# luigifcruz/radio-core

Hardware: AMD Instinct MI355X
Metric: IQ Msamples/s through Tuner+WBFM at 1024 channels (higher is better)
Workload: dtype f32

## Files before the change

### radio-core_amd/csrc/fft_kernel.h

```cpp
#pragma once

#include <hip/hip_runtime.h>

#include <cstdio>
#include <cstdlib>
#include <type_traits>

#include "fft_engine.h"
#include "tile_ns.h"

namespace rcfm {
RCFM_NS_OPEN
namespace fftk {

constexpr int W = RCFM_TILE_W;
constexpr int kLogW = W == 16 ? 4 : W == 8 ? 3 : 2;
static_assert((1 << kLogW) == W, "tile width: 4, 8 or 16 lines");
constexpr int kThreads = 256 * W / 16;

__device__ __forceinline__ float2 cmul(float2 a, float2 b) {
    typedef float v2f __attribute__((ext_vector_type(2)));
    v2f A, B, D;
    A.x = a.x; A.y = a.y; B.x = b.x; B.y = b.y;
    asm("v_pk_mul_f32 %0, %1, %2 op_sel:[0,0] op_sel_hi:[0,1]" : "=v"(D) : "v"(A), "v"(B));
// ... 765 lines not shown
    constexpr int kZeroFrom = kZeroQ > 0 && kZeroQ < R0 ? kZeroQ * (L / R0) : L;
    __shared__ __attribute__((aligned(16))) float2 tile[L * kRowsPitch];
    __shared__ __attribute__((aligned(16))) float2 tw[L];
    const FftPass& p1 = d1.p;
    const FftPass& p2 = d2.p;
    const int tid = threadIdx.x;
    const int w = tid & (W - 1), rg = tid >> kLogW;

    LineId id;
    const BlockPos bp = block_pos();
    id.batch = bp.batch;
    id.o1 = 0;
    id.o2 = 0;
    const int i0 = (int)bp.tile * W;
    const int left = (int)p1.n_inner - i0;
    const int wvalid = left < W ? left : W;
    const int64_t in_base = (int64_t)id.batch * d1.in_batch + (int64_t)i0 * p1.in_i;
    const int64_t mid_base = (int64_t)id.batch * d1.out_batch + i0;
    const int64_t out_base = (int64_t)id.batch * d2.out_batch + i0;
    const unsigned in_i = (unsigned)p1.in_i, mid_k = (unsigned)p1.out_k, out_k = (unsigned)p2.out_k;

    auto kbase = [](int g) -> int {
        if constexpr (S == 2) {
            return g;
        } else if constexpr (S == 3) {
            constexpr int w1 = L / (R0 * RL);
            const int q1 = g / w1, q2 = g - q1 * w1;
            return q1 + R0 * q2;
        } else {
            constexpr int w1 = L / (R0 * RL), w2 = L / (R0 * R1 * RL);
            const int q1 = g / w1, r1 = g - q1 * w1;
            const int q2 = r1 / w2, q3 = r1 - q2 * w2;
            return q1 + R0 * (q2 + R1 * q3);
        }
    };

    float2 v[nld];
#pragma unroll
    for (int it = 0; it < nld; ++it) {
        int e = tid + T * it;
        if ((L * W) % T != 0) e = e < L * W ? e : 0;
        const int wl = e / L, l = e - wl * L;
        const int wc = wl < wvalid ? wl : 0;
        id.i = i0 + wc;
        v[it] = load.fetch(id, l, in_base, (unsigned)wc * in_i + (unsigned)l);
    }
    float aux[nitL * RL];
    {
        const int wc = w < wvalid ? w : 0;
        id.i = i0 + wc;
#pragma unroll
        for (int it = 0; it < nitL; ++it) {
            int g = rg + RG * it;
            if (rowsL % RG != 0) g = g < rowsL ? g : 0;
            const int kb = kbase(g);
#pragma unroll
            for (int q = 0; q < RL; ++q) {
                const int k = kb + (L / RL) * q;
                aux[it * RL + q] = mid.fetch_aux(id, k, mid_base, (unsigned)k * mid_k + (unsigned)wc);
            }
        }
    }
    for (int e = tid; e < L; e += T) tw[e] = d1.stage_tw[e];

#pragma unroll
    for (int it = 0; it < nld; ++it) {
        const int e = tid + T * it;
        const int wl = e / L, l = e - wl * L;
        id.i = i0 + wl;
        float2 x = load.post(id, l, v[it]);
        if ((L * W) % T == 0 || e < L * W) tile[lds_slot<true>(l, wl)] = x;
    }
    lds_barrier();
    stage_lds<L, R0, L, true, RG>(tile, tw, w, rg);
    lds_barrier();
    if constexpr (S >= 3) {
        stage_lds<L, R1, L / R0, true, RG>(tile, tw, w, rg);
        lds_barrier();
    }
    if constexpr (S >= 4) {
        stage_lds<L, R2, L / (R0 * R1), true, RG>(tile, tw, w, rg);
        lds_barrier();
    }

    id.i = i0 + w;
    float2 xr[nitL * RL];
#pragma unroll
    for (int it = 0; it < nitL; ++it) {
        const int g = rg + RG * it;
        if ((rowsL % RG == 0) || g < rowsL) {
#pragma unroll
            for (int q = 0; q < RL; ++q) xr[it * RL + q] = tile[lds_slot<true>(g * RL + q, w)];
            dft_p<RL>(&xr[it * RL]);
        }
    }
    lds_barrier();
#pragma unroll
    for (int it = 0; it < nitL; ++it) {
        const int g = rg + RG * it;
        if ((rowsL % RG == 0) || g < rowsL) {
            const int kb = kbase(g);
#pragma unroll
            for (int q = 0; q < RL; ++q) {
                const int k = kb + (L / RL) * q;
                if constexpr (mid_upper_rows_zero<MidOp>::value) {
                    if ((L / RL) * q > L / 2) {
                        if ((L / RL) * q < kZeroFrom) tile[lds_slot<true>(k, w)] = make_float2(0.f, 0.f);
                        continue;
                    }
                }
                float2 y = mid(id, k, xr[it * RL + dft_slot<RL>(q)], aux[it * RL + q]);
                tile[lds_slot<true>(k, w)] = y;
            }
        }
    }
    lds_barrier();

    stage_lds<L, R0, L, true, RG, true, false, kZeroQ>(tile, tw, w, rg);
    lds_barrier();
    if constexpr (S >= 3) {
        stage_lds<L, R1, L / R0, true, RG>(tile, tw, w, rg);
        lds_barrier();
    }
    if constexpr (S >= 4) {
        stage_lds<L, R2, L / (R0 * R1), true, RG>(tile, tw, w, rg);
        lds_barrier();
    }
    const bool lane_ok = w < wvalid;
    const unsigned f = (unsigned)((int64_t)(i0 + w) * p2.tw_i);
    const float2 D = big_twiddle(d2, f * (unsigned)(L / RL));
#pragma unroll
    for (int it = 0; it < nitL; ++it) {
        const int g = rg + RG * it;
        if ((rowsL % RG == 0) || g < rowsL) {
            float2 x[RL];
#pragma unroll
            for (int q = 0; q < RL; ++q) x[q] = tile[lds_slot<true>(g * RL + q, w)];
            dft_p<RL>(x);
            const int kb = kbase(g);
            float2 Tw = big_twiddle(d2, f * (unsigned)kb);
            if (lane_ok) {
#pragma unroll
                for (int q = 0; q < RL; ++q) {
                    const int k = kb + (L / RL) * q;
                    const float2 y = cmul(x[dft_slot<RL>(q)], Tw);
                    Tw = cmul(Tw, D);
                    store(id, k, out_base, (unsigned)k * out_k + (unsigned)w, y);
                }
            }
        }
    }
}

template <int L, int R0, int R1, int R2, int R3, int T, class LoadOp, class MidOp, class StoreOp>
__global__ __launch_bounds__(T, (T * 16 / W >= 512 ? 4 : 1)) void k_fft_tile2_pair(FftPassDev d1, FftPassDev d2, LoadOp load,
                                                                          MidOp mid, StoreOp store, int count) {
    constexpr int S = (R0 > 1) + (R1 > 1) + (R2 > 1) + (R3 > 1);
    static_assert(S >= 2 && R0 * R1 * R2 * R3 == L, "bad radix list");
    constexpr int RL = (S == 2) ? R1 : (S == 3) ? R2 : R3;
    constexpr int RG = T / W;
    constexpr int nld = (L * W + T - 1) / T;
    constexpr int rowsL = L / RL, nitL = (rowsL + RG - 1) / RG;
    __shared__ __attribute__((aligned(16))) float2 tile[L * kRowsPitch];
    __shared__ __attribute__((aligned(16))) float2 tw[L];
    const FftPass& p1 = d1.p;
    const FftPass& p2 = d2.p;
    const int tid = threadIdx.x;
    const int w = tid & (W - 1), rg = tid >> kLogW;

    LineId id;
    const BlockPos bp = block_pos();
    id.batch = bp.batch;
    id.o1 = 0;
    id.o2 = 0;
    const int c0 = 2 * (int)bp.batch;
    const bool has1 = c0 + 1 < count;
    const int c1 = has1 ? c0 + 1 : c0;
    const int i0 = (int)bp.tile * W;
    const int left = (int)p1.n_inner - i0;
    const int wvalid = left < W ? left : W;
    const int64_t in_base = (int64_t)id.batch * d1.in_batch + (int64_t)i0 * p1.in_i;
    const int blk16 = mid.blk16;
    const int64_t mid_tile = blk16 ? (int64_t)(i0 >> 4) * blk16 + (i0 & 15) : (int64_t)i0;
    const int64_t mid_base0 = (int64_t)c0 * (blk16 ? mid.stride : d1.out_batch) + mid_tile;
    const int64_t mid_base1 = (int64_t)c1 * (blk16 ? mid.stride : d1.out_batch) + mid_tile;
    const int64_t out_base0 = (int64_t)c0 * d2.out_batch + i0;
    const int64_t out_base1 = (int64_t)c1 * d2.out_batch + i0;
    const unsigned in_i = (unsigned)p1.in_i, mid_k = blk16 ? 16u : (unsigned)p1.out_k, out_k = (unsigned)p2.out_k;
    const int wc = w < wvalid ? w : 0;

    auto lane_off = [&](int it) -> unsigned {
        int g = rg + RG * it;
        if (rowsL % RG != 0) g = g < rowsL ? g : 0;
        return (unsigned)last_stage_base<L, R0, R1, RL, S>(g) * mid_k + (unsigned)wc;
    };
    auto q_off = [&](int q) -> int64_t { return (int64_t)((L / RL) * q) * mid_k; };

    float2 v[nld];
#pragma unroll
    for (int it = 0; it < nld; ++it) {
        int e = tid + T * it;
        if ((L * W) % T != 0) e = e < L * W ? e : 0;
        const int wl = e / L, l = e - wl * L;
        const int wcl = wl < wvalid ? wl : 0;
        id.i = i0 + wcl;
        v[it] = load.fetch(id, l, in_base, (unsigned)wcl * in_i + (unsigned)l);
    }
    for (int e = tid; e < L; e += T) tw[e] = d1.stage_tw[e];
#pragma unroll
    for (int it = 0; it < nld; ++it) {
        const int e = tid + T * it;
        const int wl = e / L, l = e - wl * L;
        id.i = i0 + wl;
        const float2 x = load.post(id, l, v[it]);
        if ((L * W) % T == 0 || e < L * W) tile[lds_slot<true>(l, wl)] = x;
    }
    lds_barrier();
    stage_lds<L, R0, L, true, RG>(tile, tw, w, rg);
    lds_barrier();
    if constexpr (S >= 3) {
        stage_lds<L, R1, L / R0, true, RG>(tile, tw, w, rg);
        lds_barrier();
    }
    if constexpr (S >= 4) {
        stage_lds<L, R2, L / (R0 * R1), true, RG>(tile, tw, w, rg);
        lds_barrier();
    }

    using In0 = decltype(mid.fetch0(mid_base0, mid_base1, 0u));
    In0 a0[nitL * RL];
#pragma unroll
    for (int it = 0; it < nitL; ++it)
#pragma unroll
        for (int q = 0; q < RL; ++q)
            a0[it * RL + q] = mid.fetch0(mid_base0 + q_off(q), mid_base1 + q_off(q), lane_off(it));

    id.i = i0 + w;
    using Keep = typename MidOp::Keep;
    float2 u0[nitL * RL];
    Keep keep[nitL * RL];
#pragma unroll
    for (int it = 0; it < nitL; ++it) {
        const int g = rg + RG * it;
        if ((rowsL % RG == 0) || g < rowsL) {
            float2 x[RL];
#pragma unroll
            for (int q = 0; q < RL; ++q) x[q] = tile[lds_slot<true>(g * RL + q, w)];
            dft_p<RL>(x);
#pragma unroll
            for (int q = 0; q < RL; ++q)
                u0[it * RL + q] = mid.first(x[dft_slot<RL>(q)], a0[it * RL + q], keep[it * RL + q]);
        }
        __builtin_amdgcn_sched_barrier(0);
    }
    lds_barrier();
#pragma unroll
    for (int it = 0; it < nitL; ++it) {
        const int g = rg + RG * it;
        if ((rowsL % RG == 0) || g < rowsL) {
            const int kb = last_stage_base<L, R0, R1, RL, S>(g);
#pragma unroll
            for (int q = 0; q < RL; ++q) tile[lds_slot<true>(kb + (L / RL) * q, w)] = u0[it * RL + q];
        }
    }
    lds_barrier();

    const unsigned f = (unsigned)((int64_t)(i0 + w) * p2.tw_i);
    const float2 D = big_twiddle(d2, f * (unsigned)(L / RL));
    const bool lane_ok = w < wvalid;
    auto second_transform = [&](int64_t out_base) {
        stage_lds<L, R0, L, true, RG>(tile, tw, w, rg);
        lds_barrier();
        if constexpr (S >= 3) {
            stage_lds<L, R1, L / R0, true, RG>(tile, tw, w, rg);
            lds_barrier();
        }
        if constexpr (S >= 4) {
            stage_lds<L, R2, L / (R0 * R1), true, RG>(tile, tw, w, rg);
            lds_barrier();
        }
#pragma unroll
        for (int it = 0; it < nitL; ++it) {
            const int g = rg + RG * it;
            if ((rowsL % RG == 0) || g < rowsL) {
                float2 x[RL];
#pragma unroll
                for (int q = 0; q < RL; ++q) x[q] = tile[lds_slot<true>(g * RL + q, w)];
                dft_p<RL>(x);
                const int kb = last_stage_base<L, R0, R1, RL, S>(g);
                float2 Tw = big_twiddle(d2, f * (unsigned)kb);
                if (lane_ok) {
#pragma unroll
                    for (int q = 0; q < RL; ++q) {
                        const int k = kb + (L / RL) * q;
                        const float2 y = cmul(x[dft_slot<RL>(q)], Tw);
                        Tw = cmul(Tw, D);
                        store(id, k, out_base, (unsigned)k * out_k + (unsigned)w, y);
                    }
                }
            }
        }
    };

    float a1[nitL * RL];
#pragma unroll
    for (int it = 0; it < nitL; ++it)
#pragma unroll
        for (int q = 0; q < RL; ++q) a1[it * RL + q] = mid.fetch1(mid_base1 + q_off(q), lane_off(it));

    second_transform(out_base0);
    if (!has1) return;
    lds_barrier();
#pragma unroll
    for (int it = 0; it < nitL; ++it) {
        const int g = rg + RG * it;
        if ((rowsL % RG == 0) || g < rowsL) {
            const int kb = last_stage_base<L, R0, R1, RL, S>(g);
#pragma unroll
            for (int q = 0; q < RL; ++q) {
                const int k = kb + (L / RL) * q;
                tile[lds_slot<true>(k, w)] = mid.second(keep[it * RL + q], a1[it * RL + q]);
            }
        }
    }
    lds_barrier();
    second_transform(out_base1);
}

template <int L, int R0, int R1, int R2, int R3, int L2, int Q0, int Q1, int Q2, int T, class LoadOp, class WinOp, class StoreOp>
__global__ __launch_bounds__(T, (T * 16 / W >= 512 ? 4 : 1)) void k_fft_tile2_decim(FftPassDev d1, FftPassDev d2, LoadOp load,
                                                                           WinOp win, StoreOp store) {
    constexpr int S = (R0 > 1) + (R1 > 1) + (R2 > 1) + (R3 > 1);
    static_assert(S >= 2 && R0 * R1 * R2 * R3 == L, "bad radix list");
    constexpr int S2 = (Q0 > 1) + (Q1 > 1) + (Q2 > 1);
    static_assert(S2 >= 2 && Q0 * Q1 * Q2 == L2 && L2 % 2 == 0 && L2 < L, "bad short transform");
    constexpr int RL = (S == 2) ? R1 : (S == 3) ? R2 : R3;
    constexpr int QL = (S2 == 2) ? Q1 : Q2;
    constexpr int RG = T / W;
    constexpr int nld = (L * W + T - 1) / T;
    constexpr int rowsL = L / RL, nitL = (rowsL + RG - 1) / RG;
    constexpr int rows2 = L2 / QL;
    static_assert(rows2 <= RG, "short transform: one sweep");
    constexpr bool REG = S == 2 && nitL == 1 && Q0 == 4 && L2 == 4 * rowsL && RL >= 5 && L % L2 == 0;
    constexpr int nwin = REG ? 4 : (L2 * W + T - 1) / T;
    __shared__ __attribute__((aligned(16))) float2 tile[L * kRowsPitch];
    __shared__ __attribute__((aligned(16))) float2 tw[L];
    const FftPass& p1 = d1.p;
    const FftPass& p2 = d2.p;
    const int tid = threadIdx.x;
    const int w = tid & (W - 1), rg = tid >> kLogW;

    LineId id;
    const BlockPos bp = block_pos();
    id.batch = bp.batch;
    id.o1 = 0;
    id.o2 = 0;
    const int i0 = (int)bp.tile * W;
    const int left = (int)p1.n_inner - i0;
    const int wvalid = left < W ? left : W;
    const int64_t in_base = (int64_t)id.batch * d1.in_batch + (int64_t)i0 * p1.in_i;
    const int64_t out_base = (int64_t)id.batch * d2.out_batch + i0;
    const unsigned in_i = (unsigned)p1.in_i, out_k = (unsigned)p2.out_k;

    float2 v[nld];
#pragma unroll
    for (int it = 0; it < nld; ++it) {
        int e = tid + T * it;
        if ((L * W) % T != 0) e = e < L * W ? e : 0;
        const int wl = e / L, l = e - wl * L;
        const int wcl = wl < wvalid ? wl : 0;
        id.i = i0 + wcl;
        v[it] = load.fetch(id, l, in_base, (unsigned)wcl * in_i + (unsigned)l);
    }
    float wgt[nwin];
    if constexpr (REG) {
        const int g = rg < rowsL ? rg : 0;
#pragma unroll
        for (int q = 0; q < 4; ++q) wgt[q] = win.weight(id, g + rowsL * q, i0 + (w < wvalid ? w : 0));
    } else {
#pragma unroll
        for (int it = 0; it < nwin; ++it) {
            int e = tid + T * it;
            if ((L2 * W) % T != 0) e = e < L2 * W ? e : 0;
            const int wl = e & (W - 1);
            wgt[it] = win.weight(id, e >> kLogW, i0 + (wl < wvalid ? wl : 0));
        }
    }
    const unsigned f = (unsigned)((int64_t)(i0 + w) * p2.tw_i);
    const int kb2 = last_stage_base<L2, Q0, Q1, QL, S2>(rg < rows2 ? rg : 0);
    const float2 seedD = big_twiddle_seed(d2, f * (unsigned)rows2);
    const float2 seedT = big_twiddle_seed(d2, f * (unsigned)kb2);
    float2 tw2 = make_float2(0.f, 0.f);
    if constexpr (REG && S2 == 3) {
        static_assert(L2 <= T, "short stage table: one entry per thread");
        tw2 = d2.stage_tw[tid < L2 ? tid : 0];
    }
    for (int e = tid; e < L; e += T) tw[e] = d1.stage_tw[e];
#pragma unroll
    for (int it = 0; it < nld; ++it) {
        const int e = tid + T * it;
        const int wl = e / L, l = e - wl * L;
        id.i = i0 + wl;
        const float2 x = load.post(id, l, v[it]);
        if ((L * W) % T == 0 || e < L * W) tile[lds_slot<true>(l, wl)] = x;
    }
    lds_barrier();
    stage_lds<L, R0, L, true, RG>(tile, tw, w, rg);
    lds_barrier();
    if constexpr (S >= 3) {
        stage_lds<L, R1, L / R0, true, RG>(tile, tw, w, rg);
        lds_barrier();
    }
    if constexpr (S >= 4) {
        stage_lds<L, R2, L / (R0 * R1), true, RG>(tile, tw, w, rg);
        lds_barrier();
    }

    float2 xr[nitL * RL];
#pragma unroll
    for (int it = 0; it < nitL; ++it) {
        const int g = rg + RG * it;
        if ((rowsL % RG == 0) || g < rowsL) {
#pragma unroll
            for (int q = 0; q < RL; ++q) xr[it * RL + q] = tile[lds_slot<true>(g * RL + q, w)];
            dft_p<RL>(&xr[it * RL]);
        }
    }
    if constexpr (REG) {
        float2 y[4];
        if (rg < rowsL) {
            y[0] = xr[dft_slot<RL>(0)];
            y[1] = xr[dft_slot<RL>(1)];
            y[2] = xr[dft_slot<RL>(RL - 2)];
            y[3] = xr[dft_slot<RL>(RL - 1)];
            const bool first = rg == 0 && i0 + w == 0;
            if (first) y[2] = cadd(y[2], xr[dft_slot<RL>(2)]);
#pragma unroll
            for (int q = 0; q < 4; ++q) y[q] = make_float2(y[q].x * wgt[q], y[q].y * wgt[q]);
            if (first) {
                id.i = 0;
                win.dc_bin(id, y[0]);
            }
#pragma unroll
            for (int q = 0; q < 4; ++q) y[q] = make_float2(y[q].y, y[q].x);
            dft4(y[0], y[1], y[2], y[3]);
#pragma unroll
            for (int q = 1; q < 4; ++q) y[q] = cmul(y[q], tw[(L / L2) * q * rg]);
        }
        lds_barrier();
        if (rg < rowsL) {
#pragma unroll
            for (int q = 0; q < 4; ++q) tile[lds_slot<true>(rg + rowsL * q, w)] = y[q];
        }
        if constexpr (S2 == 3) {
            if (tid < L2) tw[tid] = tw2;
        }
        lds_barrier();
    } else {
        lds_barrier();
#pragma unroll
        for (int it = 0; it < nitL; ++it) {
            const int g = rg + RG * it;
            if ((rowsL % RG == 0) || g < rowsL) {
                const int kb = last_stage_base<L, R0, R1, RL, S>(g);
#pragma unroll
                for (int q = 0; q < RL; ++q) {
                    if ((L / RL) * q > L2 / 2 && (L / RL) * (q + 1) <= L - L2 / 2) continue;
                    const int k = kb + (L / RL) * q;
                    int l = -1;
                    if (k < L2 / 2) l = k;
                    else if (k >= L - L2 / 2) l = k - (L - L2);
                    else if (k == L2 / 2) l = L2;
                    if (l >= 0) tile[lds_slot<true>(l, w)] = xr[it * RL + dft_slot<RL>(q)];
                }
            }
        }
        for (int e = tid; e < L2; e += T) tw[e] = d2.stage_tw[e];
        lds_barrier();

// ... 28 lines not shown
    if (rg < rows2) {
        float2 x[QL];
#pragma unroll
        for (int q = 0; q < QL; ++q) x[q] = tile[lds_slot<true>(rg * QL + q, w)];
        dft_p<QL>(x);
        const float2 D = big_twiddle(d2, f * (unsigned)rows2, seedD);
        float2 Tw = big_twiddle(d2, f * (unsigned)kb2, seedT);
        if (w < wvalid) {
#pragma unroll
            for (int q = 0; q < QL; ++q) {
                const int k = kb2 + rows2 * q;
                const float2 y = cmul(x[dft_slot<QL>(q)], Tw);
                Tw = cmul(Tw, D);
                store(id, k, out_base, (unsigned)k * out_k + (unsigned)w, y);
            }
        }
    }
}


__device__ __forceinline__ float2 stream_load(const float2* p) { return *p; }

__device__ __forceinline__ void stream_store(float2* p, float2 v) {
    if constexpr (W == 16) {
        using v2 = __attribute__((ext_vector_type(2))) float;
        v2 t;
        t.x = v.x;
        t.y = v.y;
        __builtin_nontemporal_store(t, reinterpret_cast<v2*>(p));
    } else {
        *p = v;
    }
}

template <bool SWAP>
struct LoadPlainT {
    const float2* in;
    __device__ __forceinline__ float2 fetch(const LineId&, int, int64_t base, unsigned off) const {
        return stream_load(in + base + off);
    }
    __device__ __forceinline__ float2 post(const LineId&, int, float2 v) const {
        return SWAP ? make_float2(v.y, v.x) : v;
    }
};

__device__ __forceinline__ float2 iq_bits(unsigned raw) { return make_float2(__uint_as_float(raw), 0.f); }

struct LoadIq16 {
    const uint32_t* in;
    __device__ __forceinline__ float2 fetch(const LineId&, int, int64_t base, unsigned off) const {
        return iq_bits(in[base + off]);
    }
    __device__ __forceinline__ float2 post(const LineId&, int, float2 v) const {
        const unsigned raw = __float_as_uint(v.x);
        return make_float2((float)(int16_t)(raw & 0xffffu) * 0x1p-15f, (float)(int16_t)(raw >> 16) * 0x1p-15f);
    }
};

struct LoadIq8 {
    const uint16_t* in;
    __device__ __forceinline__ float2 fetch(const LineId&, int, int64_t base, unsigned off) const {
        return iq_bits(in[base + off]);
    }
    __device__ __forceinline__ float2 post(const LineId&, int, float2 v) const {
        const unsigned raw = __float_as_uint(v.x);
        return make_float2((float)(int8_t)(raw & 0xffu) * 0x1p-7f, (float)(int8_t)(raw >> 8) * 0x1p-7f);
    }
};

struct LoadIqU8 {
    const uint16_t* in;
    __device__ __forceinline__ float2 fetch(const LineId&, int, int64_t base, unsigned off) const {
        return iq_bits(in[base + off]);
    }
    __device__ __forceinline__ float2 post(const LineId&, int, float2 v) const {
        const unsigned raw = __float_as_uint(v.x);
        return make_float2(((float)(raw & 0xffu) - 127.5f) * 0x1p-7f, ((float)(raw >> 8) - 127.5f) * 0x1p-7f);
    }
};

template <bool SWAP>
struct StorePlainT {
    float2* out;
    float scale;
    __device__ __forceinline__ void operator()(const LineId&, int, int64_t base, unsigned off, float2 v) const {
        stream_store(out + base + off,
                     SWAP ? make_float2(v.y * scale, v.x * scale) : make_float2(v.x * scale, v.y * scale));
    }
};

struct StoreRowWindow {
    float2* out;
    float scale;
    int n_o1, n_o2, lo, hi;
    int64_t n = 0;
    int halo = 0;
    int sc1_straddle = 0;
    __device__ __forceinline__ void operator()(const LineId& id, int k, int64_t base, unsigned off, float2 v) const {
        const int row = (int)id.o1 + n_o1 * ((int)id.o2 + n_o2 * k);
        const bool keep = lo <= hi ? (row >= lo && row <= hi) : (row >= lo || row <= hi);
        if (!keep) return;
        const float2 y = make_float2(v.x * scale, v.y * scale);
        const int64_t g = base + off;
        const bool straddle = sc1_straddle &&
                              ((reinterpret_cast<uintptr_t>(out + g) - ((uintptr_t)((int)id.i & (W - 1)) << 3)) & 127u) != 0;
        if (straddle) asm volatile("global_store_dwordx2 %0, %1, off sc1" : : "v"(out + g), "v"(y) : "memory");
        else stream_store(out + g, y);
        if (halo > 0) {
            if (g < halo) out[n + g] = y;
            else if (g >= n - halo) out[g - n] = y;
        }
    }
};

}
RCFM_NS_CLOSE
}
namespace rcfm {
RCFM_NS_OPEN
namespace fftk {

#define RCFM_FFT_LONG_TABLE3(X) X(480, 10, 8, 6, 1) X(500, 10, 10, 5, 1)
#define RCFM_FFT_LONG_TABLE(X) X(480, 24, 20, 1, 1) X(500, 25, 20, 1, 1)
#ifndef RCFM_R640
#define RCFM_R640 10, 8, 8, 1
#endif
#ifndef RCFM_R600
#define RCFM_R600 10, 10, 6, 1
#endif
#define RCFM_FFT_BIG_X_(X, LEN, ...) X(LEN, __VA_ARGS__)
#define RCFM_FFT_BIG_LENGTHS(X) RCFM_FFT_BIG_X_(X, 600, RCFM_R600) X(625, 5, 5, 5, 5) RCFM_FFT_BIG_X_(X, 640, RCFM_R640)
#define RCFM_FFT_LENGTHS_(X, LONGT) \
    X(75, 5, 5, 3, 1)            \
    X(80, 10, 8, 1, 1)           \
    X(100, 10, 10, 1, 1)         \
    X(120, 12, 10, 1, 1)         \
    X(125, 5, 5, 5, 1)           \
    X(128, 8, 8, 2, 1)           \
    X(150, 15, 10, 1, 1)         \
    X(160, 16, 10, 1, 1)         \
    X(192, 16, 12, 1, 1)         \
    X(200, 20, 10, 1, 1)         \
    X(240, 24, 10, 1, 1)         \
    X(250, 25, 10, 1, 1)         \
    X(256, 16, 16, 1, 1)         \
    X(300, 20, 15, 1, 1)         \
    X(320, 10, 8, 4, 1)          \
    X(375, 5, 5, 5, 3)           \
    X(384, 8, 8, 6, 1)           \
    X(400, 20, 20, 1, 1)         \
    LONGT(X)                     \
    X(512, 8, 8, 8, 1)
#define RCFM_FFT_FAST_LENGTHS(X) RCFM_FFT_LENGTHS_(X, RCFM_FFT_LONG_TABLE)
#define RCFM_FFT_PAIR_LENGTHS(X) RCFM_FFT_LENGTHS_(X, RCFM_FFT_LONG_TABLE3)


constexpr int tile_threads(int L) {
    return (big_tile_pair(L) ? 1024 : L >= 320 ? 512 : 256) * W / 16;
}

template <class T> struct is_plain_functor : std::false_type {};
template <bool S> struct is_plain_functor<LoadPlainT<S>> : std::true_type {};
template <bool S> struct is_plain_functor<StorePlainT<S>> : std::true_type {};
template <> struct is_plain_functor<LoadIq16> : std::true_type {};
template <> struct is_plain_functor<LoadIq8> : std::true_type {};
template <> struct is_plain_functor<LoadIqU8> : std::true_type {};
template <> struct is_plain_functor<StoreRowWindow> : std::true_type {};

enum PassKinds : int { kAnyPass = 0, kStridedOnly = 1, kRowsOnly = 2 };

template <int LEN, int A, int B, int C, int D, bool ROWS, class LoadOp, class StoreOp>
inline void launch_fft_tile_one(const FftPassDev& d, dim3 grid, const LoadOp& ld, const StoreOp& st, hipStream_t s) {
    constexpr int T = tile_threads(LEN);
    hipLaunchKernelGGL((k_fft_tile<LEN, A, B, C, D, ROWS, T, LoadOp, StoreOp>), grid, dim3(T), 0, s, d, ld, st);
}

template <int KIND = kAnyPass, class LoadOp, class StoreOp>
inline void launch_fft_pass(const FftPassDev& d, int batch, const LoadOp& ld, const StoreOp& st, hipStream_t s) {
    bool done = false;
    const bool rows = d.p.load_along_l != 0;
    RC_REQUIRE(!(KIND == kStridedOnly && rows) && !(KIND == kRowsOnly && !rows), RCFM_ERR_RUNTIME,
               "FFT functor used with the wrong pass kind");
    const bool shape_ok = (rows || d.p.in_i == 1) && d.p.out_i == 1 && ((d.p.has_twiddle != 0) == !rows) &&
                          d.p.n_o1 * d.p.n_o2 <= 65535 && batch <= 65535;
    if (shape_ok) {
        const unsigned tiles_inner = (unsigned)((d.p.n_inner + W - 1) / W), outer = (unsigned)(d.p.n_o1 * d.p.n_o2);
        const dim3 grid = d.p.flat_outer ? dim3((tiles_inner * outer + 7u) / 8u * 8u, 1, (unsigned)batch)
                                         : dim3(tiles_inner, outer, (unsigned)batch);
        switch (d.p.L) {
#define RCFM_CASE(LEN, A, B, C, D)                                                                            \
    case LEN:                                                                                                 \
        if (rows) {                                                                                           \
            if constexpr (KIND != kStridedOnly)                                                               \
                launch_fft_tile_one<LEN, A, B, C, D, true, LoadOp, StoreOp>(d, grid, ld, st, s);               \
        } else {                                                                                              \
            if constexpr (KIND != kRowsOnly)                                                                  \
                launch_fft_tile_one<LEN, A, B, C, D, false, LoadOp, StoreOp>(d, grid, ld, st, s);              \
        }                                                                                                     \
        done = true;                                                                                          \
        break;
            RCFM_FFT_FAST_LENGTHS(RCFM_CASE)
            default: break;
        }
        if constexpr (W == 16 && is_plain_functor<LoadOp>::value && is_plain_functor<StoreOp>::value) {
            switch (d.p.L) {
                RCFM_FFT_BIG_LENGTHS(RCFM_CASE)
                default: break;
            }
        }
#undef RCFM_CASE
    }
    if (!done)
        hipLaunchKernelGGL((k_fft_pass<LoadOp, StoreOp>),
                           dim3((unsigned)(d.p.n_o1 * d.p.n_o2 * ((d.p.n_inner + W - 1) / W)), (unsigned)batch, 1),
                           dim3(kThreads), (size_t)d.p.L * (W * sizeof(float2) + sizeof(float2) + sizeof(uint16_t)), s, d,
                           ld, st);
    RC_HIP(hipGetLastError());
}

inline bool fft_tile2_applies(const FftPassDev& d1, const FftPassDev& d2, int batch) {
    bool fast = false;
    switch (d1.p.L) {
#define RCFM_CASE(LEN, A, B, C, D) case LEN:
        RCFM_FFT_FAST_LENGTHS(RCFM_CASE)
#undef RCFM_CASE
        fast = true;
        break;
        default: break;
    }
    return fast && d1.p.load_along_l && !d2.p.load_along_l && d1.p.L == d2.p.L &&
           d1.p.n_inner == d2.p.n_inner && d1.p.n_o1 * d1.p.n_o2 == 1 && d2.p.n_o1 * d2.p.n_o2 == 1 &&
           d1.p.out_k == d2.p.in_l && d2.p.in_i == 1 && d2.p.out_i == 1 && d2.p.has_twiddle && batch <= 65535;
}

#ifndef RCFM_DECIM_100
#define RCFM_DECIM_100 4, 5, 5
#endif
#define RCFM_FFT_DECIM_X_(X, ...) X(__VA_ARGS__)
#define RCFM_FFT_DECIM_500(X) RCFM_FFT_DECIM_X_(X, 500, 25, 20, 1, 1, 100, RCFM_DECIM_100)
#define RCFM_FFT_DECIM_125(X) X(125, 5, 5, 5, 1, 80, 10, 8, 1)
#define RCFM_FFT_DECIM_PAIRS(X)          \
    RCFM_FFT_DECIM_500(X)                \
    RCFM_FFT_DECIM_125(X)

inline bool fft_tile2_decim_applies(const FftPassDev& d1, const FftPassDev& d2, int batch) {
    bool fast = false;
#define RCFM_CASE(LEN, A, B, C, D, LEN2, E, F, G) fast = fast || (d1.p.L == LEN && d2.p.L == LEN2);
    RCFM_FFT_DECIM_PAIRS(RCFM_CASE)
#undef RCFM_CASE
    return fast && d1.p.load_along_l && !d2.p.load_along_l &&
           d1.p.n_inner == d2.p.n_inner && d1.p.n_o1 * d1.p.n_o2 == 1 && d2.p.n_o1 * d2.p.n_o2 == 1 &&
           d1.p.out_k == d2.p.in_l && d2.p.in_i == 1 && d2.p.out_i == 1 && d2.p.has_twiddle && batch <= 65535;
}

template <class LoadOp, class WinOp, class StoreOp>
inline bool launch_fft_tile2_decim(const FftPassDev& d1, const FftPassDev& d2, int batch, const LoadOp& ld,
                                   const WinOp& win, const StoreOp& st, hipStream_t s) {
    if (!fft_tile2_decim_applies(d1, d2, batch)) return false;
    const dim3 grid((unsigned)((d1.p.n_inner + W - 1) / W), 1, (unsigned)batch);
    bool done = false;
#define RCFM_CASE(LEN, A, B, C, D, LEN2, E, F, G)                                                                \
    if (!done && d1.p.L == LEN && d2.p.L == LEN2) {                                                             \
        hipLaunchKernelGGL((k_fft_tile2_decim<LEN, A, B, C, D, LEN2, E, F, G, tile_threads(LEN), LoadOp, WinOp, StoreOp>), \
                           grid, dim3(tile_threads(LEN)), 0, s, d1, d2, ld, win, st);                           \
        done = true;                                                                                            \
    }
    RCFM_FFT_DECIM_PAIRS(RCFM_CASE)
#undef RCFM_CASE
    if (!done) return false;
    RC_HIP(hipGetLastError());
    return true;
}

template <class LoadOp, class MidOp, class StoreOp>
inline bool launch_fft_tile2_pair(const FftPassDev& d1, const FftPassDev& d2, int count, const LoadOp& ld,
                                  const MidOp& mid, const StoreOp& st, hipStream_t s) {
    const int pairs = (count + 1) / 2;
    if (!fft_tile2_applies(d1, d2, pairs)) return false;
    const dim3 grid((unsigned)((d1.p.n_inner + W - 1) / W), 1, (unsigned)pairs);
    switch (d1.p.L) {
#define RCFM_CASE(LEN, A, B, C, D)                                                                               \
    case LEN:                                                                                                    \
        hipLaunchKernelGGL((k_fft_tile2_pair<LEN, A, B, C, D, tile_threads(LEN), LoadOp, MidOp, StoreOp>), grid, \
                           dim3(tile_threads(LEN)), 0, s, d1, d2, ld, mid, st, count);                           \
        break;
        RCFM_FFT_PAIR_LENGTHS(RCFM_CASE)
#undef RCFM_CASE
        default: return false;
    }
    RC_HIP(hipGetLastError());
    return true;
}

template <class LoadOp, class MidOp, class StoreOp>
inline bool launch_fft_tile2(const FftPassDev& d1, const FftPassDev& d2, int batch, const LoadOp& ld,
                             const MidOp& mid, const StoreOp& st, hipStream_t s) {
    if (!fft_tile2_applies(d1, d2, batch)) return false;
    const dim3 grid((unsigned)((d1.p.n_inner + W - 1) / W), 1, (unsigned)batch);
    switch (d1.p.L) {
#define RCFM_CASE(LEN, A, B, C, D)                                                                           \
    case LEN:                                                                                                \
        hipLaunchKernelGGL((k_fft_tile2<LEN, A, B, C, D, tile_threads(LEN), LoadOp, MidOp, StoreOp>), grid,  \
                           dim3(tile_threads(LEN)), 0, s, d1, d2, ld, mid, st);                              \
        break;
        RCFM_FFT_FAST_LENGTHS(RCFM_CASE)
#undef RCFM_CASE
        default: return false;
// ... 9 lines not shown
```

### radio-core_amd/csrc/fused_passes.hip

```cpp
#include "fused_passes.h"
#include "device_math.h"

#include "fft_kernel.h"
#include "fft_decim_rt.h"
#include "kernels.h"

namespace rcfm {
RCFM_NS_OPEN

using fftk::LineId;
using fftk::kAnyPass;
using fftk::kRowsOnly;
using fftk::kStridedOnly;

namespace {


struct LoadTunerGatherFast {
    const float2* X;
    const int32_t* base;
    float two_pi_over_n, delta;
    float c0, c1, c2, c3;
    int B, nyq;
    int merge;
// ... 141 lines not shown
        return make_float2(phase_step_wrapped(a.x, b.x), phase_step_wrapped(a.y, b.y));
    }
};

LoadPhaseStepPair phase_pair_load(const float* x, int64_t n, int count, int line_stride, const PhaseRows& r) {
    LoadPhaseStepPair ld{x, (int)n, count, line_stride};
    ld.stride = r.channel_stride(n);
    if (r.row > 0 && r.pitch > r.row) {
        RC_REQUIRE(n % r.row == 0 && n < (1 << 20) && r.row < (1 << 12), RCFM_ERR_RUNTIME, "phase rows outside the reader's range");
        ld.row = r.row;
        ld.pad = r.pitch - r.row;
        ld.magic = (unsigned)((((uint64_t)1 << 32) + (uint64_t)r.row - 1) / (uint64_t)r.row);
    }
    return ld;
}

template <bool HZ>
struct LoadHilbertPairT {
    static constexpr int kFetches = 2;
    static constexpr bool kHalfZones = HZ;
    const float2* U;
    int n;
    int line_stride;
    __device__ __forceinline__ const float2* pair(const LineId& id) const {
        return U + (int64_t)(id.batch >> 1) * n;
    }
    __device__ __forceinline__ float2 fetch(const LineId& id, int l, int64_t, unsigned, int zone = 1) const {
        const int k = l * line_stride + (int)id.i;
        return pair(id)[(zone == 0 || k <= n / 2) ? k : 0];
    }
    __device__ __forceinline__ float2 fetch2(const LineId& id, int l, int64_t, unsigned, int zone = 1) const {
        const int k = l * line_stride + (int)id.i;
        return pair(id)[((zone == 0 || k <= n / 2) && k > 0) ? n - k : 0];
    }
    __device__ __forceinline__ float2 post(const LineId& id, int l, float2 a, float2 b, int zone = 1) const {
        const int k = l * line_stride + (int)id.i;
        float h = (k == 0) ? 0.5f : 1.f;
        if (zone != 0) {
            if (k >= (n + 1) / 2) h = 0.f;
            if ((n & 1) == 0 && k == n / 2) h = 0.5f;
        }
        float2 xk;
        if ((id.batch & 1) == 0) xk = make_float2(a.x + b.x, a.y - b.y);
        else xk = make_float2(a.y + b.y, -(a.x - b.x));
        return make_float2(xk.y * h, xk.x * h);
    }
};

template <bool HZ>
struct LoadHilbertPackedT {
    static constexpr bool kHalfZones = HZ;
    const float2* U2;
    int n;
    int line_stride;
    float scale;
    __device__ __forceinline__ float2 fetch(const LineId& id, int l, int64_t, unsigned, int zone = 1) const {
        const int k = l * line_stride + (int)id.i;
        return (U2 + (int64_t)id.batch * n)[(zone == 0 || k <= n / 2) ? k : 0];
    }
    __device__ __forceinline__ float2 post(const LineId& id, int l, float2 v, int zone = 1) const {
        const int k = l * line_stride + (int)id.i;
        float h = (k == 0) ? scale : 2.f * scale;
        if (zone != 0) {
            if (k >= (n + 1) / 2) h = 0.f;
            if ((n & 1) == 0 && k == n / 2) h = scale;
        }
        return make_float2(v.y * h, v.x * h);
    }
};

template <class Launch>
void with_hilbert_pair_load(const FftEngine& e, const float2* U, Launch&& launch) {
    const FftPass& p = e.desc().pass[0];
    const int64_t n = e.desc().n;
    if (e.npass() == 2 && !p.load_along_l && p.in_l * p.L == n && p.L % 2 == 0)
        launch(LoadHilbertPairT<true>{U, (int)n, (int)p.in_l});
    else
        launch(LoadHilbertPairT<false>{U, (int)n, (int)p.in_l});
}

struct LoadHilbertMask {
    const float2* U;
    int n;
    int64_t line_stride;
    __device__ __forceinline__ float2 fetch(const LineId& id, int, int64_t base, unsigned off) const {
        const int64_t cbase = (int64_t)id.batch * n;
        const int64_t a = base + off;
        return U[(a - cbase) <= n / 2 ? a : cbase];
    }
    __device__ __forceinline__ float2 post(const LineId& id, int l, float2 v) const {
        const int k = (int)(l * line_stride + id.i);
        float h = 0.f;
        if (k == 0) h = 1.f;
        else if (k < (n + 1) / 2) h = 2.f;
        else if ((n & 1) == 0 && k == n / 2) h = 1.f;
        return make_float2(v.y * h, v.x * h);
    }
};

__device__ __forceinline__ float pilot_carrier(float a, float b) {
    return (2.f * a * b) * __builtin_amdgcn_rcpf(fmaf(a, a, b * b));
}
__device__ __forceinline__ float2 stereo_mix_point(float2 v, float mm) {
    const float s2 = pilot_carrier(v.y, v.x);
    const float lmr = (s2 * mm) * 1.0175f;
    return make_float2(mm + lmr, mm - lmr);
}

struct StoreStereoMix {
    static constexpr bool kAux = true;
    const float* m;
    float2* u;
    __device__ __forceinline__ float fetch_aux(const LineId&, int, int64_t base, unsigned off) const {
        return (m + base)[off];
    }
    __device__ __forceinline__ void operator()(const LineId&, int, int64_t base, unsigned off, float2 v,
                                               float mm) const {
        fftk::stream_store(u + base + off, stereo_mix_point(v, mm));
    }
};

struct MidStereoMix {
    [[maybe_unused]] static constexpr bool kAux = true;
    const float* m;
    __device__ __forceinline__ float fetch_aux(const LineId&, int, int64_t base, unsigned off) const {
        return (m + base)[off];
    }
    __device__ __forceinline__ float2 operator()(const LineId&, int, float2 v, float mm) const {
        return stereo_mix_point(v, mm);
    }
};

template <bool UPPER_ZERO>
struct MidHilbertMaskT {
    [[maybe_unused]] static constexpr bool kAux = true;
    static constexpr bool kUpperRowsZero = UPPER_ZERO;
    int n, stride;
    float scale;
    __device__ __forceinline__ float fetch_aux(const LineId&, int, int64_t, unsigned) const { return 0.f; }
    __device__ __forceinline__ float2 operator()(const LineId& id, int k, float2 v, float) const {
        const int bin = k * stride + (int)id.i;
        float h = (bin == 0) ? scale : 2.f * scale;
        if (bin >= (n + 1) / 2) h = 0.f;
        if ((n & 1) == 0 && bin == n / 2) h = scale;
        return make_float2(v.y * h, v.x * h);
    }
};

struct MidStereoMixPair {
    const float* p;
    const float* m;
    int64_t stride = 0;
    int blk16 = 0;
    struct In0 { float p0, p1, m0; };
    using Keep = float;
    static __device__ __forceinline__ float at(const float* base, unsigned off) {
        return *reinterpret_cast<const float*>(reinterpret_cast<const char*>(base) + (size_t)(off * 4u));
    }
    __device__ __forceinline__ In0 fetch0(int64_t b0, int64_t b1, unsigned off) const {
        return In0{at(p + b0, off), at(p + b1, off), at(m + b0, off)};
    }
    __device__ __forceinline__ float fetch1(int64_t b1, unsigned off) const { return at(m + b1, off); }
    __device__ __forceinline__ float2 first(float2 v, const In0& a, Keep& s2_1) const {
        s2_1 = pilot_carrier(a.p1, a.p0 - v.y);
        const float lmr = (pilot_carrier(a.p0, v.x - a.p1) * a.m0) * 1.0175f;
        return make_float2(a.m0 + lmr, a.m0 - lmr);
    }
    __device__ __forceinline__ float2 second(const Keep& s2_1, float m1) const {
        const float lmr = (s2_1 * m1) * 1.0175f;
        return make_float2(m1 + lmr, m1 - lmr);
    }
};

struct LoadStereoUnpack {
    static constexpr int kFetches = 3;
    const float2* U;
    const float* wr;
    float2* dc;
    int B, A, nyq, nmin;
    float nyq_factor, scale;
    int line_stride;
    __device__ __forceinline__ int folded(int k) const { return k > A / 2 ? A - k : k; }
    __device__ __forceinline__ float2 fetch(const LineId& id, int l, int64_t, unsigned) const {
        const int kk = folded(l * line_stride + (int)id.i);
        return (U + (int64_t)id.batch * B)[kk < nyq ? kk : 0];
    }
    __device__ __forceinline__ float2 fetch2(const LineId& id, int l, int64_t, unsigned) const {
        const int kk = folded(l * line_stride + (int)id.i);
        return (U + (int64_t)id.batch * B)[(kk < nyq && kk > 0) ? B - kk : 0];
    }
    __device__ __forceinline__ float fetch3(const LineId& id, int l, int64_t, unsigned) const {
        const int kk = folded(l * line_stride + (int)id.i);
        return wr[kk < nyq ? kk : 0];
    }
    __device__ __forceinline__ float2 post(const LineId& id, int l, float2 a, float2 b, float w0) const {
        const int k = l * line_stride + (int)id.i;
        const bool mirrored = k > A / 2;
        const int kk = mirrored ? A - k : k;
        float2 hl = make_float2(0.f, 0.f), hr = make_float2(0.f, 0.f);
        if (kk < nyq) {
            float w = w0 * scale;
            if ((nmin & 1) == 0 && kk == nmin / 2) w *= nyq_factor;
            hl = make_float2(0.5f * (a.x + b.x) * w, 0.5f * (a.y - b.y) * w);
            hr = make_float2(0.5f * (a.y + b.y) * w, -0.5f * (a.x - b.x) * w);
            if (kk == 0 || ((A & 1) == 0 && kk == A / 2)) {
                hl.y = 0.f;
                hr.y = 0.f;
            }
        }
        if (mirrored) {
            hl.y = -hl.y;
            hr.y = -hr.y;
        }
        const float2 out = make_float2(hl.x - hr.y, hl.y + hr.x);
        if (k == 0 && dc != nullptr) dc[id.batch] = out;
        return make_float2(out.y, out.x);
    }
};


struct StorePruned {
    float2* out;
    int n, lo, hi;
    StorePruned(float2* o, int n_, int keep) : out(o), n(n_) {
        if (keep == kKeepLowerHalf) {
            lo = n_ / 2;
            hi = n_ + 1;
        } else if (keep < 0) {
            lo = n_;
            hi = 0;
        } else {
            lo = keep;
            hi = n_ - keep;
        }
    }
    __device__ __forceinline__ void operator()(const LineId& id, int, int64_t base, unsigned off, float2 v) const {
        const int k = (int)(base + off - (int64_t)id.batch * n);
        if (k <= lo || k >= hi) fftk::stream_store(out + base + off, v);
    }
};

struct StoreRealPart {
    float* y;
    float scale;
    __device__ __forceinline__ void operator()(const LineId&, int, int64_t base, unsigned off, float2 v) const {
        (y + base)[off] = v.y * scale;
    }
};

void middle_passes(const FftEngine& e, int from, int to, float2* tmp, int count, hipStream_t s) {
    const int64_t ts = e.tmp_stride();
    for (int t = from; t <= to; ++t) {
        fftk::LoadPlainT<false> ld{tmp};
        fftk::StorePlainT<false> st{tmp, 1.0f};
        fftk::launch_fft_pass<kStridedOnly>(e.pass_dev(t, ts, ts), count, ld, st, s);
    }
}

}

struct StorePhase {
    float* theta;
    __device__ __forceinline__ void operator()(const LineId&, int, int64_t base, unsigned off, float2 v) const {
        (theta + base)[off] = atan2_over_pi(v.x, v.y);
    }
};

struct StoreEnvelope {
    float* e;
    float scale;
    __device__ __forceinline__ void operator()(const LineId&, int, int64_t base, unsigned off, float2 v) const {
        const float re = v.y * scale, im = v.x * scale;
        (e + base)[off] = sqrtf(re * re + im * im);
    }
};

void fused_tuner_ifft(const FftEngine& e, const TunerGather& g, float2* out, float2* tmp, int count,
                      hipStream_t s, float* theta, int theta_pitch, bool envelope) {
    if (count <= 0) return;
    const int64_t B = e.desc().n;
    const int np = e.npass();
    fftk::StorePlainT<false> st0{tmp, 1.0f};
    auto first_pass = [&](auto ld) {
        ld.X = g.X;
        ld.roll = g.roll;
        ld.N = (decltype(ld.N))g.N;
        ld.two_pi_over_n = (float)(6.28318530717958647692 / (double)g.N);
        ld.delta = (g.N % 2) ? (float)(3.14159265358979323846 / (double)g.N) : 0.f;
        ld.a0 = (float)g.a0;
        ld.B = (int)B;
        ld.nyq = g.nyq;
        ld.nneg = g.nneg;
        ld.nyq_mode = g.nyq_mode;
        ld.line_stride = (int)e.desc().pass[0].in_l;
        ld.x_batch = g.x_batch;
        fftk::launch_fft_pass<kStridedOnly>(e.pass_dev(0, 0, e.tmp_stride()), count, ld, st0, s);
    };
    const bool series = 6.28318530717958647692 * ((double)(B / 2 + 2) / (double)g.N) < 0.25;
    if (series && g.base32 && g.halo >= B / 2 + 1 && g.nyq_mode != NYQ_UP && B <= g.N && g.x_batch == 0) {
        LoadTunerGatherFast ld;
        const double a1 = 1.0 - g.a0;
        ld.X = g.X;
        ld.base = g.base32;
        ld.two_pi_over_n = (float)(6.28318530717958647692 / (double)g.N);
        ld.delta = (g.N % 2) ? (float)(3.14159265358979323846 / (double)g.N) : 0.f;
        ld.c0 = (float)(g.a0 + a1);
        ld.c1 = (float)(-a1 / 2.0);
        ld.c2 = (float)(a1 / 24.0);
        ld.c3 = (float)(-a1 / 720.0);
        ld.B = (int)B;
        ld.nyq = g.nyq;
        ld.merge = g.nyq_mode == NYQ_DOWN ? g.nyq - 1 : -1;
        ld.line_stride = (int)e.desc().pass[0].in_l;
        fftk::launch_fft_pass<kStridedOnly>(e.pass_dev(0, 0, e.tmp_stride()), count, ld, st0, s);
    } else if (g.N >= (int64_t)1 << 30) {
        first_pass(LoadTunerGatherT<int64_t, false>{});
    } else {
        first_pass(LoadTunerGatherT<int32_t, false>{});
    }
    middle_passes(e, 1, np - 2, tmp, count, s);
    fftk::LoadPlainT<false> ldl{tmp};
    if (theta != nullptr) {
        FftPassDev last = e.pass_dev(np - 1, e.tmp_stride(), B);
// ... 419 lines not shown
```

Before: 35040.

## Defer mono fetches in paired stereo FFT kernel to cut register pressure

Restructures the paired stereo-mix FFT kernel. The mono sample for the first channel is now fetched after the first-stage DFT, and the second channel's mono fetch moves to just after the first stage of the second transform. Both changes shorten the live ranges of loaded values and let global loads overlap LDS work. It also switches the pair kernel's long-length radix table from the 3-stage variant to the default table. The cost is more compile-time configuration paths and a different stage count for long lengths.

New measurement: 35460, median of 6. 1.2% higher.

```diff
diff --git a/radio-core_amd/csrc/fft_kernel.h b/radio-core_amd/csrc/fft_kernel.h
--- a/radio-core_amd/csrc/fft_kernel.h
+++ b/radio-core_amd/csrc/fft_kernel.h
@@ -941,6 +941,13 @@
     }
 }
 
+#ifndef RCFM_PAIR_FORM
+#define RCFM_PAIR_FORM 2
+#endif
+#ifndef RCFM_PAIR_M1_AFTER
+#define RCFM_PAIR_M1_AFTER 1
+#endif
+constexpr bool pair_late_fetch(int ) { return RCFM_PAIR_FORM != 0; }
 template <int L, int R0, int R1, int R2, int R3, int T, class LoadOp, class MidOp, class StoreOp>
 __global__ __launch_bounds__(T, (T * 16 / W >= 512 ? 4 : 1)) void k_fft_tile2_pair(FftPassDev d1, FftPassDev d2, LoadOp load,
                                                                           MidOp mid, StoreOp store, int count) {
@@ -1016,40 +1023,86 @@
         lds_barrier();
     }
 
+    constexpr bool LATE = pair_late_fetch(L);
     using In0 = decltype(mid.fetch0(mid_base0, mid_base1, 0u));
+    using Keep = typename MidOp::Keep;
     In0 a0[nitL * RL];
-#pragma unroll
-    for (int it = 0; it < nitL; ++it)
-#pragma unroll
-        for (int q = 0; q < RL; ++q)
-            a0[it * RL + q] = mid.fetch0(mid_base0 + q_off(q), mid_base1 + q_off(q), lane_off(it));
-
+    float m0[nitL * RL];
+    Keep keep[nitL * RL];
     id.i = i0 + w;
-    using Keep = typename MidOp::Keep;
-    float2 u0[nitL * RL];
-    Keep keep[nitL * RL];
-#pragma unroll
-    for (int it = 0; it < nitL; ++it) {
-        const int g = rg + RG * it;
-        if ((rowsL % RG == 0) || g < rowsL) {
-            float2 x[RL];
-#pragma unroll
-            for (int q = 0; q < RL; ++q) x[q] = tile[lds_slot<true>(g * RL + q, w)];
-            dft_p<RL>(x);
+    if constexpr (LATE) {
+#pragma unroll
+        for (int it = 0; it < nitL; ++it)
 #pragma unroll
             for (int q = 0; q < RL; ++q)
-                u0[it * RL + q] = mid.first(x[dft_slot<RL>(q)], a0[it * RL + q], keep[it * RL + q]);
-        }
-        __builtin_amdgcn_sched_barrier(0);
-    }
-    lds_barrier();
-#pragma unroll
-    for (int it = 0; it < nitL; ++it) {
-        const int g = rg + RG * it;
-        if ((rowsL % RG == 0) || g < rowsL) {
-            const int kb = last_stage_base<L, R0, R1, RL, S>(g);
-#pragma unroll
-            for (int q = 0; q < RL; ++q) tile[lds_slot<true>(kb + (L / RL) * q, w)] = u0[it * RL + q];
+                a0[it * RL + q] = mid.fetch0(mid_base0 + q_off(q), mid_base1 + q_off(q), lane_off(it));
+
+        Keep keep0[nitL * RL];
+#pragma unroll
+        for (int it = 0; it < nitL; ++it) {
+            const int g = rg + RG * it;
+            if ((rowsL % RG == 0) || g < rowsL) {
+                float2 x[RL];
+#pragma unroll
+                for (int q = 0; q < RL; ++q) x[q] = tile[lds_slot<true>(g * RL + q, w)];
+                dft_p<RL>(x);
+#pragma unroll
+                for (int q = 0; q < RL; ++q)
+                    mid.first(x[dft_slot<RL>(q)], a0[it * RL + q], keep0[it * RL + q], keep[it * RL + q]);
+            }
+            __builtin_amdgcn_sched_barrier(0);
+        }
+#pragma unroll
+        for (int it = 0; it < nitL; ++it)
+#pragma unroll
+            for (int q = 0; q < RL; ++q) m0[it * RL + q] = mid.fetch1(mid_base0 + q_off(q), lane_off(it));
+        lds_barrier();
+#pragma unroll
+        for (int it = 0; it < nitL; ++it) {
+            const int g = rg + RG * it;
+            if ((rowsL % RG == 0) || g < rowsL) {
+                const int kb = last_stage_base<L, R0, R1, RL, S>(g);
+#pragma unroll
+                for (int q = 0; q < RL; ++q)
+                    tile[lds_slot<true>(kb + (L / RL) * q, w)] = mid.second(keep0[it * RL + q], m0[it * RL + q]);
+            }
+        }
+    } else {
+#pragma unroll
+        for (int it = 0; it < nitL; ++it)
+#pragma unroll
+            for (int q = 0; q < RL; ++q) {
+                a0[it * RL + q] = mid.fetch0(mid_base0 + q_off(q), mid_base1 + q_off(q), lane_off(it));
+                m0[it * RL + q] = mid.fetch1(mid_base0 + q_off(q), lane_off(it));
+            }
+
+        float2 u0[nitL * RL];
+#pragma unroll
+        for (int it = 0; it < nitL; ++it) {
+            const int g = rg + RG * it;
+            if ((rowsL % RG == 0) || g < rowsL) {
+                float2 x[RL];
+#pragma unroll
+                for (int q = 0; q < RL; ++q) x[q] = tile[lds_slot<true>(g * RL + q, w)];
+                dft_p<RL>(x);
+#pragma unroll
+                for (int q = 0; q < RL; ++q) {
+                    Keep k0;
+                    mid.first(x[dft_slot<RL>(q)], a0[it * RL + q], k0, keep[it * RL + q]);
+                    u0[it * RL + q] = mid.second(k0, m0[it * RL + q]);
+                }
+            }
+            __builtin_amdgcn_sched_barrier(0);
+        }
+        lds_barrier();
+#pragma unroll
+        for (int it = 0; it < nitL; ++it) {
+            const int g = rg + RG * it;
+            if ((rowsL % RG == 0) || g < rowsL) {
+                const int kb = last_stage_base<L, R0, R1, RL, S>(g);
+#pragma unroll
+                for (int q = 0; q < RL; ++q) tile[lds_slot<true>(kb + (L / RL) * q, w)] = u0[it * RL + q];
+            }
         }
     }
     lds_barrier();
@@ -1057,8 +1110,9 @@
     const unsigned f = (unsigned)((int64_t)(i0 + w) * p2.tw_i);
     const float2 D = big_twiddle(d2, f * (unsigned)(L / RL));
     const bool lane_ok = w < wvalid;
-    auto second_transform = [&](int64_t out_base) {
+    auto second_transform = [&](int64_t out_base, auto&& after_first_stage) {
         stage_lds<L, R0, L, true, RG>(tile, tw, w, rg);
+        after_first_stage();
         lds_barrier();
         if constexpr (S >= 3) {
             stage_lds<L, R1, L / R0, true, RG>(tile, tw, w, rg);
@@ -1091,13 +1145,20 @@
         }
     };
 
+    constexpr bool M1_AFTER = LATE && RCFM_PAIR_M1_AFTER;
     float a1[nitL * RL];
-#pragma unroll
-    for (int it = 0; it < nitL; ++it)
-#pragma unroll
-        for (int q = 0; q < RL; ++q) a1[it * RL + q] = mid.fetch1(mid_base1 + q_off(q), lane_off(it));
-
-    second_transform(out_base0);
+    auto fetch_a1 = [&]() {
+#pragma unroll
+        for (int it = 0; it < nitL; ++it)
+#pragma unroll
+            for (int q = 0; q < RL; ++q) a1[it * RL + q] = mid.fetch1(mid_base1 + q_off(q), lane_off(it));
+    };
+    if constexpr (M1_AFTER) {
+        second_transform(out_base0, fetch_a1);
+    } else {
+        fetch_a1();
+        second_transform(out_base0, [] {});
+    }
     if (!has1) return;
     lds_barrier();
 #pragma unroll
@@ -1113,7 +1174,7 @@
         }
     }
     lds_barrier();
-    second_transform(out_base1);
+    second_transform(out_base1, [] {});
 }
 
 template <int L, int R0, int R1, int R2, int R3, int L2, int Q0, int Q1, int Q2, int T, class LoadOp, class WinOp, class StoreOp>
@@ -1448,7 +1509,12 @@
     LONGT(X)                     \
     X(512, 8, 8, 8, 1)
 #define RCFM_FFT_FAST_LENGTHS(X) RCFM_FFT_LENGTHS_(X, RCFM_FFT_LONG_TABLE)
-#define RCFM_FFT_PAIR_LENGTHS(X) RCFM_FFT_LENGTHS_(X, RCFM_FFT_LONG_TABLE3)
+#if RCFM_PAIR_FORM >= 2
+#define RCFM_FFT_PAIR_LONG RCFM_FFT_LONG_TABLE
+#else
+#define RCFM_FFT_PAIR_LONG RCFM_FFT_LONG_TABLE3
+#endif
+#define RCFM_FFT_PAIR_LENGTHS(X) RCFM_FFT_LENGTHS_(X, RCFM_FFT_PAIR_LONG)
 
 
 constexpr int tile_threads(int L) {
diff --git a/radio-core_amd/csrc/fused_passes.hip b/radio-core_amd/csrc/fused_passes.hip
--- a/radio-core_amd/csrc/fused_passes.hip
+++ b/radio-core_amd/csrc/fused_passes.hip
@@ -317,23 +317,22 @@
     const float* m;
     int64_t stride = 0;
     int blk16 = 0;
-    struct In0 { float p0, p1, m0; };
+    struct In0 { float p0, p1; };
     using Keep = float;
     static __device__ __forceinline__ float at(const float* base, unsigned off) {
         return *reinterpret_cast<const float*>(reinterpret_cast<const char*>(base) + (size_t)(off * 4u));
     }
     __device__ __forceinline__ In0 fetch0(int64_t b0, int64_t b1, unsigned off) const {
-        return In0{at(p + b0, off), at(p + b1, off), at(m + b0, off)};
-    }
-    __device__ __forceinline__ float fetch1(int64_t b1, unsigned off) const { return at(m + b1, off); }
-    __device__ __forceinline__ float2 first(float2 v, const In0& a, Keep& s2_1) const {
+        return In0{at(p + b0, off), at(p + b1, off)};
+    }
+    __device__ __forceinline__ float fetch1(int64_t b, unsigned off) const { return at(m + b, off); }
+    __device__ __forceinline__ void first(float2 v, const In0& a, Keep& s2_0, Keep& s2_1) const {
         s2_1 = pilot_carrier(a.p1, a.p0 - v.y);
-        const float lmr = (pilot_carrier(a.p0, v.x - a.p1) * a.m0) * 1.0175f;
-        return make_float2(a.m0 + lmr, a.m0 - lmr);
-    }
-    __device__ __forceinline__ float2 second(const Keep& s2_1, float m1) const {
-        const float lmr = (s2_1 * m1) * 1.0175f;
-        return make_float2(m1 + lmr, m1 - lmr);
+        s2_0 = pilot_carrier(a.p0, v.x - a.p1);
+    }
+    __device__ __forceinline__ float2 second(const Keep& s2, float mm) const {
+        const float lmr = (s2 * mm) * 1.0175f;
+        return make_float2(mm + lmr, mm - lmr);
     }
 };
 
```
